# microsoft/NOTSOFAR1-Challenge

Hardware: AMD Instinct MI355X
Metric: CSS real-time-factor (sep. audio sec/wall sec) on 7-ch 16 kHz (higher is better)
Workload: dtype f32 (float32 operands on v_mfma_f32_32x32x2_f32 in every Linear layer, attention product and transform: the reference's own operand precision; MVDR covariance / solve f64)

## Files before the change

### notsofar1-challenge_amd/csrc/api_core.hip

```cpp
#include "api_ctx.hpp"

thread_local std::string g_create_error;

int fail(css_ctx* h, int code, const std::string& msg) {
    if (h) h->err = msg;
    else g_create_error = msg;
    return code;
}

hipError_t dev_alloc(DevBuf& b, size_t bytes) {
    hipError_t e = b.reset();
    if (e == hipSuccess) e = hipMalloc(&b.p, bytes);
    if (e == hipSuccess) b.cap = bytes;
    return e;
}

int ensure(css_ctx* h, DevBuf& b, size_t bytes, bool zero) {
    if (bytes <= b.cap) return CSS_OK;
    if (b.p && h->queued) HIPCHK(h, hipDeviceSynchronize());
    if (const hipError_t e = b.reset()) return fail(h, CSS_ERR_HIP, std::string("hipFree(b.p): ") + hipGetErrorString(e));
    HIPCHK(h, hipMalloc(&b.p, bytes));
    b.cap = bytes;
    if (zero) HIPCHK(h, hipMemsetAsync(b.p, 0, bytes, h->stream));
    return CSS_OK;
// ... 97 lines not shown
    bool ok = true;
    for (int k = 0; k < 20 && ok && !enough(); ++k) {
        hipStream_t st = nullptr;
        if (hipStreamCreateWithFlags(&st, hipStreamNonBlocking) != hipSuccess) { ok = false; break; }
        if (streams_share_a_queue(main, st, e0, e1)) { with_main.push_back(st); continue; }
        bool placed = false;
        for (auto& c : cls)
            if (streams_share_a_queue(c[0], st, e0, e1)) { c.push_back(st); placed = true; break; }
        if (!placed) cls.push_back({st});
    }
    e0.reset();
    e1.reset();
    if (hipGetLastError() != hipSuccess) ok = false;
    std::vector<hipStream_t> take;
    if (ok && !cls.empty()) {
        std::sort(cls.begin(), cls.end(), [](const std::vector<hipStream_t>& x, const std::vector<hipStream_t>& y) { return x.size() > y.size(); });
        auto pop = [&](size_t c) -> hipStream_t {
            for (size_t q = 0; q < cls.size(); ++q) {
                auto& v = cls[(c + q) % cls.size()];
                if (!v.empty()) { hipStream_t s_ = v.back(); v.pop_back(); return s_; }
            }
            if (!with_main.empty()) { hipStream_t s_ = with_main.back(); with_main.pop_back(); return s_; }
            return nullptr;
        };
        const size_t nc = cls.size();
        const size_t cA = 0, cB = nc > 1 ? 1 : 0, cC = nc > 2 ? 2 : cB;
        take.resize(5);
        take[2] = pop(cC);
        take[0] = pop(cA);
        take[1] = pop(cB);
        take[3] = pop(cB);
        take[4] = pop(cA);
        for (hipStream_t s_ : take) ok = ok && s_ != nullptr;
    } else {
        ok = false;
    }
    for (auto& c : cls)
        for (hipStream_t s_ : c) hipStreamDestroy(s_);
    for (hipStream_t s_ : with_main) hipStreamDestroy(s_);
    if (!ok) {
        for (hipStream_t s_ : take)
            if (s_) hipStreamDestroy(s_);
        return false;
    }
    lane[1] = take[0]; lane[2] = take[1]; *copy = take[2]; *tail = take[3]; lane[3] = take[4];
    return true;
}

int plan_impl(const CssModelDesc& d, const CssRunCfg& cfg, int64_t n, CssPlan* p) {
    const int T = cfg.segment_frames, hop = cfg.hop_frames;
    if (T <= 0 || hop <= 0 || hop > T) return CSS_ERR_INVALID_ARG;
    p->n_samples = n;
    p->stft_frames = n < d.frame_len ? 0 : (n - d.frame_len) / d.frame_hop + 1;
    p->mix_frames = std::max<int64_t>(p->stft_frames, T);
    const int64_t ov = T - hop;
    p->num_segments = (p->mix_frames - ov + hop - 1) / hop;
    p->n_out = (p->mix_frames - 1) * d.frame_hop + d.frame_len;
    const int64_t st = (p->num_segments - 1) * hop;
    int64_t en = st + T;
    if (en >= p->mix_frames) en = p->mix_frames;
    p->last_valid = (int32_t)(en - st);
    p->zero_weight = 0;
    if (cfg.w_first && cfg.w_mid && cfg.w_last) {
        for (int64_t t = 0; t < p->mix_frames && !p->zero_weight; ++t) {
            float ws = 0.f;
            for (int64_t seg = std::max<int64_t>(0, (t - T + hop) / hop); seg <= t / hop && seg < p->num_segments; ++seg) {
                const int64_t tl = t - seg * hop;
                if (tl < 0 || tl >= T) continue;
                const float* w = seg == 0 ? cfg.w_first : (seg == p->num_segments - 1 ? cfg.w_last : cfg.w_mid);
                ws += w[tl];
            }
            if (!(ws > 1e-5f)) p->zero_weight = 1;
        }
    }
    return CSS_OK;
}

void gemm(css_ctx* h, const GemmArgs& g, hipStream_t st) {
    CSS_PROF(CSS_PROF_LINEAR, st);
    if (h->profile_gemm) h->gemm_flops += 2.0 * g.M * (double)g.N * g.K * g.batch;
    if (!g.split_in && !g.layout && h->tune[CSS_TUNE_F32_GEMM]) {
        GemmArgs q = g;
        const int t = h->tune[CSS_TUNE_F32_GEMM];
        q.layout = t == 1 ? 2 : (t == 6 ? 1 : 10 + std::min(t - 1, 4));
        launch_gemm(q, st);
        return;
    }
    launch_gemm(g, st);
}

GemmArgs linear(const float* A, int64_t lda, const float* W, int64_t ldw, const float* bias, float* C, int64_t ldc,
                int M, int N, int K, int act) {
    GemmArgs g{};
    g.A = A; g.lda = lda; g.strideA = 0;
    g.B = W; g.ldb = ldw; g.strideB = 0;
    g.C = C; g.ldc = ldc; g.strideC = 0;
    g.M = M; g.N = N; g.K = K; g.batch = 1;
    g.bias = bias; g.bias_along_m = 0; g.act = act;
    g.residual = nullptr; g.ldr = 0; g.alpha = 1.f;
    return g;
}

StitchArgs stitch_args(css_ctx* h) {
    StitchArgs a{};
    const int T = h->cfg.segment_frames;
    a.masks = h->masks_v;
    a.mask_ld = h->mask_ld_v;
    a.sep = (const float*)h->sep.p;
    a.S = h->d.num_spks; a.F = h->d.num_bins; a.T = T; a.hop = h->cfg.hop_frames;
    a.num_segments = h->plan.num_segments; a.T_long = h->plan.mix_frames;
    a.w_first = (const float*)h->segw.p; a.w_mid = a.w_first + T; a.w_last = a.w_mid + T;
    a.perms = (const int32_t*)h->perms.p;
    a.mask_st = (float*)h->mask_st.p; a.activity = (float*)h->activity.p;
    a.act_b = (uint8_t*)h->act_b.p; a.act_tmp = (uint8_t*)h->act_tmp.p; a.act_final = (uint8_t*)h->act_final.p;
    a.activity_th = h->cfg.activity_th; a.dilation = h->cfg.dilation_frames; a.erosion = h->cfg.erosion_frames;
    a.Y = (float*)h->Y.p; a.KIp = h->KIp;
    a.y_split = h->split ? 1 : 0;
    a.level = h->split ? h->peak_dev : nullptr;
    return a;
}

MvdrArgs mvdr_args(css_ctx* h, int64_t lo, int nseg) {
    MvdrArgs a{};
    const int T = h->cfg.segment_frames;
    a.X = (const float*)h->X.p; a.T_ld = h->T_ld; a.stft_frames = h->plan.stft_frames;
    a.C = h->n_ch; a.F = h->d.num_bins;
    a.masks = h->masks_v; a.mask_ld = h->mask_ld_v;
    a.S = h->d.num_spks; a.T = T; a.hop = h->cfg.hop_frames;
    a.seg_lo = lo; a.nseg = nseg;
    a.wta_override = h->have_override ? (const uint8_t*)h->wta.p : nullptr;
    a.scm = (double*)h->scm.p; a.bfw = (double*)h->bfw.p; a.sep = (float*)h->sep.p;
    a.mask_floor = h->cfg.mask_floor;
    a.use_mvdr = (h->n_ch > 1 && h->cfg.mc_mvdr) ? 1 : 0;
    return a;
}

int64_t batch_cap(const css_ctx* h, int T) {
    int64_t cap = h->max_batch;
    const int rows = h->tune[CSS_TUNE_SPLIT_BATCH_ROWS];
    if (h->split && rows > 0 && T > 0) cap = std::min<int64_t>(cap, std::max<int64_t>(1, rows / T));
    return cap;
}

int ensure_activations(css_ctx* h, int64_t nb, int T) {
    const int64_t Mb = nb * T;
    const int D = h->d.attention_dim, FF = h->d.linear_units;
    int rc;
    if ((rc = ensure(h, h->feat, (size_t)Mb * h->Kp * sizeof(float), true)) != CSS_OK) return rc;
    if ((rc = ensure(h, h->hx, (size_t)Mb * D * sizeof(float))) != CSS_OK) return rc;
    if ((rc = ensure(h, h->hu, (size_t)Mb * D * sizeof(float))) != CSS_OK) return rc;
    if ((rc = ensure(h, h->ht, (size_t)Mb * FF * sizeof(float))) != CSS_OK) return rc;
    if ((rc = ensure(h, h->qkv, (size_t)Mb * 3 * D * sizeof(float))) != CSS_OK) return rc;
    if ((rc = ensure(h, h->qkf, (size_t)qk_fragment_floats(nb, T, h->d.attention_heads) * sizeof(float), true)) != CSS_OK) return rc;
    if ((rc = ensure(h, h->ctxb, (size_t)Mb * D * sizeof(float))) != CSS_OK) return rc;
    for (int l = 1; l < h->lanes; ++l) {
        const int64_t M2 = ((nb + 1) / 2) * T;
        if ((rc = ensure(h, h->lfeat[l], (size_t)M2 * h->Kp * sizeof(float), true)) != CSS_OK) return rc;
        if ((rc = ensure(h, h->lhx[l], (size_t)M2 * D * sizeof(float))) != CSS_OK) return rc;
        if ((rc = ensure(h, h->lhu[l], (size_t)M2 * D * sizeof(float))) != CSS_OK) return rc;
        if ((rc = ensure(h, h->lht[l], (size_t)M2 * FF * sizeof(float))) != CSS_OK) return rc;
        if ((rc = ensure(h, h->lqkv[l], (size_t)M2 * 3 * D * sizeof(float))) != CSS_OK) return rc;
        if ((rc = ensure(h, h->lqkf[l], (size_t)qk_fragment_floats(M2 / T, T, h->d.attention_heads) * sizeof(float), true)) != CSS_OK) return rc;
        if ((rc = ensure(h, h->lctx[l], (size_t)M2 * D * sizeof(float))) != CSS_OK) return rc;
    }
    return CSS_OK;
}

// ... 288 lines not shown
    if (!h || lanes < 1 || lanes > css_ctx::MAX_LANES) return fail(h, CSS_ERR_INVALID_ARG, "lanes must be in [1, 4]");
    h->lanes = lanes;
    return CSS_OK;
}

int css_get_lanes(css_handle_t h) { return h ? h->lanes : (int)CSS_ERR_INVALID_ARG; }

int css_set_tuning(css_handle_t h, int which, int value) {
    if (!h || which < 0 || which >= CSS_TUNE_COUNT || value < 0 || (value > 16 && which != CSS_TUNE_SPLIT_BATCH_ROWS && which != CSS_TUNE_F32_LANE_ROWS))
        return fail(h, CSS_ERR_INVALID_ARG, "unknown tuning option / value");
    h->tune[which] = value;
    return CSS_OK;
}

int css_set_range_fallback(css_handle_t h, int enable) {
    if (!h) return CSS_ERR_INVALID_ARG;
    h->range_fallback = enable != 0;
    return CSS_OK;
}

int css_range_status(css_handle_t h, int64_t* fallbacks, int32_t* last_hit) {
    if (!h) return CSS_ERR_INVALID_ARG;
    if (fallbacks) *fallbacks = h->range_fallbacks;
    if (last_hit) *last_hit = h->range_last;
    return CSS_OK;
}

int css_check_range(css_handle_t h) {
    int rc = check_session(h);
    if (rc) return rc;
    HIPCHK(h, hipSetDevice(h->device));
    HIPCHK(h, hipMemcpyAsync(h->range_flag_host.p, h->range_flag_dev.p, sizeof(unsigned int), hipMemcpyDeviceToHost, h->stream));
    HIPCHK(h, hipStreamSynchronize(h->stream));
    if (*h->range_flag_host.as<unsigned int>() && h->split)
        return fail(h, CSS_ERR_RANGE, "an operand of a Linear layer left the split-f16 range (|x| > 65504): use CSS_LINEAR_EXACT_F32");
    return CSS_OK;
}

int css_linear_host(css_handle_t h, const float* x, const float* w, const float* bias, int32_t M, int32_t N, int32_t K,
                    int32_t kernel, int32_t layout, float* y) {
    CSS_DRAIN(h);
    if (!h || !x || !w || !y || M < 1 || N < 1 || K < 32 || K % 32) return fail(h, CSS_ERR_INVALID_ARG, "bad argument (K must be a multiple of 32)");
    if (kernel < 0 || kernel > 2) return fail(h, CSS_ERR_INVALID_ARG, "kernel must be 0 (split, weights direct), 1 (split, LDS staged) or 2 (exact float32)");
    HIPCHK(h, hipSetDevice(h->device));
    const int Np = (N + 31) / 32 * 32;
    const size_t xf = (size_t)M * K, wf = (size_t)Np * K, yf = (size_t)M * N;
    int rc;
    if ((rc = ensure(h, h->stage, (2 * xf + 2 * wf + yf + (size_t)N + 256) * sizeof(float))) != CSS_OK) return rc;
    float* xd = (float*)h->stage.p;
    float* xs = xd + (xf + 15) / 16 * 16;
    float* wd = xs + (xf + 15) / 16 * 16;
    float* ws = wd + (wf + 15) / 16 * 16;
    float* yd = ws + (wf + 15) / 16 * 16;
    float* bd = yd + (yf + 15) / 16 * 16;
    HIPCHK(h, hipMemcpyAsync(xd, x, xf * sizeof(float), hipMemcpyHostToDevice, h->stream));
    HIPCHK(h, hipMemcpyAsync(wd, w, (size_t)N * K * sizeof(float), hipMemcpyHostToDevice, h->stream));
    if (bias) HIPCHK(h, hipMemcpyAsync(bd, bias, (size_t)N * sizeof(float), hipMemcpyHostToDevice, h->stream));
    GemmArgs g = linear(xd, K, wd, K, bias ? bd : nullptr, yd, N, M, N, K, ACT_NONE);
    if (kernel != 2) {
        launch_split_convert(xd, K, xs, M, K, K, h->stream);
        if (kernel == 0) launch_split_convert_tiled(wd, K, ws, N, K, h->stream);
        else launch_split_convert(wd, K, ws, N, K, K, h->stream);
        g.A = xs; g.B = ws; g.split_in = 1; g.b_tiled = kernel == 0;
        if (kernel == 0) g.tile_rows = layout; else g.layout = layout;
    } else {
        g.layout = layout;
    }
    launch_gemm(g, h->stream);
    HIPCHK(h, hipMemcpyAsync(y, yd, yf * sizeof(float), hipMemcpyDeviceToHost, h->stream));
    HIPCHK(h, hipStreamSynchronize(h->stream));
    HIPCHK(h, hipGetLastError());
    return CSS_OK;
}

int css_gemm_host(css_handle_t h, const CssGemmDesc* d, const float* a, const float* b, const float* bias, const float* residual,
                  float* c) {
    CSS_DRAIN(h);
    if (!h) return CSS_ERR_INVALID_ARG;
    auto bad = [&](const char* what) { return fail(h, CSS_ERR_INVALID_ARG, std::string("css_gemm_host: ") + what); };
    if (!d || !a || !b || !c) return bad("null argument");
    const int64_t cap = (int64_t)1 << 28;
    const int M = d->M, N = d->N, K = d->K, batch = d->batch, kernel = d->kernel;
    if (kernel < 0 || kernel > 2) return bad("kernel must be 0 (split, weights direct), 1 (split, LDS staged) or 2 (exact float32)");
    if (M < 1 || N < 1 || batch < 1 || K < 32 || K % 32 || M > (1 << 22) || N > (1 << 22) || K > (1 << 16) || batch > 1024)
        return bad("M, N, batch >= 1 and K a multiple of 32");
    if (d->lda < K || d->ldb < K || d->lda % 4 || d->ldb % 4 || d->lda > cap || d->ldb > cap) return bad("lda, ldb: multiples of 4, at least K");
    if (d->act < ACT_NONE || d->act > ACT_SIGMOID) return bad("act must be 0, 1 or 2");
    if (d->bias < 0 || d->bias > 2 || (d->bias != 0) != (bias != nullptr)) return bad("bias: 0 with NULL, 1 or 2 with an array");
    if (d->residual < 0 || d->residual > 2 || (d->residual == 1) != (residual != nullptr)) return bad("residual: 1 with an array, 0 or 2 with NULL");
    if (!(std::fabs(d->alpha) <= 3.0e38f)) return bad("alpha must be finite");
    if (d->a_off < 0 || d->c_off < 0 || d->r_off < 0 || d->a_off > 1024 || d->c_off > (1 << 20) || d->r_off > 1024) return bad("offsets");
    const bool tr = d->c_transposed != 0, has_res = d->residual != 0;
    const int rows_c = tr ? N : M, cols_c = tr ? M : N;
    if (d->ldc < cols_c || d->ldc > cap) return bad("ldc is shorter than a row of C");
    const int64_t ldr = d->residual == 2 ? d->ldc : d->ldr;
    if (d->residual == 1 && (ldr < N || ldr > cap)) return bad("ldr is shorter than a row of the residual");
    if (d->residual == 2 && batch != 1) return bad("the in-place residual takes batch 1");
    const int64_t extA = (int64_t)(M - 1) * d->lda + K, extB = (int64_t)(N - 1) * d->ldb + K;
    const int64_t extC = (int64_t)(rows_c - 1) * d->ldc + cols_c, extR = (int64_t)(M - 1) * ldr + N;
    const int64_t sA = batch > 1 ? d->strideA : 0, sB = batch > 1 ? d->strideB : 0, sC = batch > 1 ? d->strideC : 0;
    if (sA < 0 || sB < 0 || sA > cap || sB > cap || sC > cap || (sA && sA < extA) || (sB && sB < extB)) return bad("strideA, strideB: 0 or at least one matrix");
    if (batch > 1 && sC < extC) return bad("batch entries of C overlap");
    if (d->a_floats > cap || d->b_floats > cap || d->c_floats > cap || d->r_floats > cap) return bad("an array of more than 2^28 floats");
    if (d->a_floats < d->a_off + (batch - 1) * sA + extA) return bad("a is shorter than its description");
    if (d->b_floats < (batch - 1) * sB + extB) return bad("b is shorter than its description");
    if (d->c_floats < d->c_off + (batch - 1) * sC + extC) return bad("c is shorter than its description");
    if (d->residual == 1 && d->r_floats < d->r_off + extR) return bad("residual is shorter than its description");
    if (d->split_out < 0 || d->split_out % 32 || d->split_out > N || (d->split_out && kernel == 2)) return bad("split_out: a multiple of 32 up to N, kernels 0 and 1");
    if (tr && (kernel != 0 || has_res || d->split_out || d->bias == 2)) return bad("c_transposed: kernel 0, column bias and activation only");
    if (kernel == 0 && (batch != 1 || N % 32)) return bad("kernel 0 takes batch 1 and whole 32-column weight tiles");
    if (kernel == 0 && !tr && (d->c_off % 4 || d->ldc % 4)) return bad("kernel 0 writes 16-byte pieces: c_off and ldc must be multiples of 4");
    if (d->b_frag32 && (kernel != 2 || batch != 1 || N % 32)) return bad("b_frag32: kernel 2, batch 1, N a multiple of 32");
    const int lay = d->layout, tile = d->tile_rows;
    const bool lay_ok = kernel == 0 ? lay == 0
                                    : (lay == 0 || lay == 8 || lay == 4 || lay == 64 || (kernel == 2 && (lay == 1 || lay == 2 || (lay >= 11 && lay <= 14))));
    const bool tile_ok = kernel == 0 ? (tile == 0 || tile == 32 || tile == 64 || tile == 96 || tile == 128 || tile == 4 || tile == 65) : tile == 0;
    if (!lay_ok || !tile_ok) return bad("layout / tile_rows: not a tile layout of this kernel");

    HIPCHK(h, hipSetDevice(h->device));
    auto pad = [](int64_t n) { return (size_t)((n + 63) / 64 * 64); };
    const int nA = sA ? batch : 1, nB = sB ? batch : 1;
    const int Np = (N + 31) / 32 * 32;
    const size_t f_a = pad(d->a_floats), f_b = pad(d->b_floats), f_c = pad(d->c_floats), f_r = pad(d->residual == 1 ? d->r_floats : 0);
    const size_t f_as = kernel != 2 ? pad((int64_t)nA * M * K) : 0, f_bs = kernel == 0 ? pad((int64_t)Np * K) : kernel == 1 ? pad((int64_t)nB * N * K) : 0;
    const size_t f_bf = d->b_frag32 ? pad((int64_t)N * K) : 0, f_bias = pad(d->bias == 2 ? M : N);
    int rc;
    if ((rc = ensure(h, h->stage, (f_a + f_b + f_c + f_r + f_as + f_bs + f_bf + f_bias) * sizeof(float))) != CSS_OK) return rc;
    float* ad = (float*)h->stage.p;
    float* bd = ad + f_a;
    float* cd = bd + f_b;
    float* rd = cd + f_c;
    float* as = rd + f_r;
    float* bs = as + f_as;
    float* bf = bs + f_bs;
    float* biasd = bf + f_bf;
    HIPCHK(h, hipMemcpyAsync(ad, a, (size_t)d->a_floats * sizeof(float), hipMemcpyHostToDevice, h->stream));
    HIPCHK(h, hipMemcpyAsync(bd, b, (size_t)d->b_floats * sizeof(float), hipMemcpyHostToDevice, h->stream));
    HIPCHK(h, hipMemcpyAsync(cd, c, (size_t)d->c_floats * sizeof(float), hipMemcpyHostToDevice, h->stream));
    if (d->residual == 1) HIPCHK(h, hipMemcpyAsync(rd, residual, (size_t)d->r_floats * sizeof(float), hipMemcpyHostToDevice, h->stream));
    if (bias) HIPCHK(h, hipMemcpyAsync(biasd, bias, (size_t)(d->bias == 2 ? M : N) * sizeof(float), hipMemcpyHostToDevice, h->stream));

    GemmArgs g{};
    g.A = ad + d->a_off; g.lda = d->lda; g.strideA = sA;
    g.B = bd; g.ldb = d->ldb; g.strideB = sB;
    g.C = cd + d->c_off; g.ldc = d->ldc; g.strideC = sC;
    g.M = M; g.N = N; g.K = K; g.batch = batch;
    g.bias = bias ? biasd : nullptr; g.bias_along_m = d->bias == 2; g.act = d->act;
    g.residual = d->residual == 1 ? rd + d->r_off : d->residual == 2 ? g.C : nullptr;
    g.ldr = has_res ? ldr : 0; g.alpha = has_res ? d->alpha : 1.f;
    g.split_out = d->split_out; g.c_transposed = tr; g.m_fastest = d->m_fastest != 0; g.nt_store = d->nt_store != 0;
    g.concurrent = d->concurrent != 0;
    if (kernel != 2) {
        for (int z = 0; z < nA; ++z) launch_split_convert(g.A + z * sA, d->lda, as + (int64_t)z * M * K, M, K, K, h->stream);
        if (kernel == 0) launch_split_convert_tiled(bd, d->ldb, bs, N, K, h->stream);
        else for (int z = 0; z < nB; ++z) launch_split_convert(bd + z * sB, d->ldb, bs + (int64_t)z * N * K, N, K, K, h->stream);
        g.A = as; g.lda = K; g.strideA = sA ? (int64_t)M * K : 0;
        g.B = bs; g.ldb = K; g.strideB = sB ? (int64_t)N * K : 0;
        g.split_in = 1; g.b_tiled = kernel == 0;
        g.tile_rows = tile; g.layout = lay;
    } else {
        g.layout = lay;
        if (d->b_frag32) {
            launch_f32_fragments(bd, d->ldb, bf, N, K, h->stream);
            g.B = bf; g.b_frag32 = 1; g.B_rows = bd;
        }
    }
    launch_gemm(g, h->stream);
    HIPCHK(h, hipMemcpyAsync(c, cd, (size_t)d->c_floats * sizeof(float), hipMemcpyDeviceToHost, h->stream));
    HIPCHK(h, hipStreamSynchronize(h->stream));
    HIPCHK(h, hipGetLastError());
    return CSS_OK;
}

int css_host_alloc(size_t bytes, void** out) {
    if (!out) return CSS_ERR_INVALID_ARG;
    *out = nullptr;
    return hipHostMalloc(out, bytes ? bytes : 1, hipHostMallocDefault) == hipSuccess ? CSS_OK : CSS_ERR_HIP;
}

int css_host_free(void* p) { return (!p || hipHostFree(p) == hipSuccess) ? CSS_OK : CSS_ERR_HIP; }

int css_set_linear_mode(css_handle_t h, int mode) {
    CSS_DRAIN(h);
    if (!h || (mode != CSS_LINEAR_SPLIT_F16 && mode != CSS_LINEAR_EXACT_F32)) return fail(h, CSS_ERR_INVALID_ARG, "unknown linear mode");
    const bool split = mode == CSS_LINEAR_SPLIT_F16;
    if (split == h->split) return CSS_OK;
    if (split && stream_open_count(h)) return fail(h, CSS_ERR_STATE, "a stream is open: streams run in CSS_LINEAR_EXACT_F32 only");
    if (split && !h->split_ok) return fail(h, CSS_ERR_RANGE, "a weight of this model lies outside the split-f16 operand range (|w| > 65504)");
    HIPCHK(h, hipSetDevice(h->device));
    if (split) {
        int rc = make_split_weights(h);
        if (rc) return rc;
    } else if (make_frag_weights(h) != CSS_OK) {
        (void)hipGetLastError();
        h->wfrag.reset();
    }
    if (h->feat.p) HIPCHK(h, hipMemsetAsync(h->feat.p, 0, h->feat.cap, h->stream));
    for (int l = 1; l < css_ctx::MAX_LANES; ++l)
// ... 342 lines not shown
```

### notsofar1-challenge_amd/csrc/gemm.hip

```cpp
#include <cstdlib>

#include <cstdio>

#include "gemm_common.hpp"

namespace css {

template <int BM, int WM>
__global__ __launch_bounds__(WM * 128, 2) void gemm_kernel(GemmArgs g, int tiles_m, int tiles_n) {
    constexpr int THREADS = WM * 128;
    constexpr int TM = (BM / WM) / 32;
    constexpr int LROWS = THREADS / 8;
    constexpr int NLA = BM / LROWS;
    constexpr int NLB = BN / LROWS;
    static_assert((NLA == 2 || NLA == 4) && (NLB == 2 || NLB == 4) && (TM == 1 || TM == 2), "unsupported tile layout");
    __shared__ __attribute__((aligned(16))) float lds[2 * (BM + BN) * LDS_LD];
    const int n_tiles = tiles_m * tiles_n * g.batch;
    const int L = blockIdx.x;
    const int tile = xcd_tile(L, n_tiles);
    const int per_batch = tiles_m * tiles_n;
    const int bz = tile / per_batch;
    const int t2 = tile - bz * per_batch;
    const int tn = g.m_fastest ? t2 / tiles_m : t2 % tiles_n, tm = g.m_fastest ? t2 % tiles_m : t2 / tiles_n;
    const int m0 = tm * BM, n0 = tn * BN;
// ... 37 lines not shown
#define CSS_LSTORE(buf)                                                         \
    {                                                                           \
        float* as_ = lds + (buf) * (BM + BN) * LDS_LD + lr * LDS_LD + lc;       \
        float* bs_ = as_ + BM * LDS_LD;                                         \
        *reinterpret_cast<float4*>(as_) = ra0;                                  \
        *reinterpret_cast<float4*>(as_ + LROWS * LDS_LD) = ra1;                 \
        *reinterpret_cast<float4*>(bs_) = rb0;                                  \
        *reinterpret_cast<float4*>(bs_ + LROWS * LDS_LD) = rb1;                 \
        if constexpr (NLA == 4) {                                               \
            *reinterpret_cast<float4*>(as_ + 2 * LROWS * LDS_LD) = ra2;         \
            *reinterpret_cast<float4*>(as_ + 3 * LROWS * LDS_LD) = ra3;         \
        }                                                                       \
        if constexpr (NLB == 4) {                                               \
            *reinterpret_cast<float4*>(bs_ + 2 * LROWS * LDS_LD) = rb2;         \
            *reinterpret_cast<float4*>(bs_ + 3 * LROWS * LDS_LD) = rb3;         \
        }                                                                       \
    }

    f32x16 acc00 = {0}, acc01 = {0}, acc10 = {0}, acc11 = {0};
    const int nk = g.K / BK;
    CSS_GLOAD(0)
    CSS_LSTORE(0)
    __syncthreads();
    for (int kt = 0; kt < nk; ++kt) {
        const int buf = kt & 1;
        if (kt + 1 < nk) { CSS_GLOAD((kt + 1) * BK) }
        const float* as = lds + buf * (BM + BN) * LDS_LD + (wm * (BM / WM) + c) * LDS_LD + 4 * h;
        const float* bs = lds + buf * (BM + BN) * LDS_LD + BM * LDS_LD + (wn * 64 + c) * LDS_LD + 4 * h;
#pragma unroll
        for (int ch = 0; ch < 4; ++ch) {
            const float4 a0 = *reinterpret_cast<const float4*>(as + ch * 8);
            const float4 b0 = *reinterpret_cast<const float4*>(bs + ch * 8);
            const float4 b1 = *reinterpret_cast<const float4*>(bs + 32 * LDS_LD + ch * 8);
            float4 a1 = a0;
            if constexpr (TM == 2) a1 = *reinterpret_cast<const float4*>(as + 32 * LDS_LD + ch * 8);
#define CSS_MFMA_STEP(e)                                                                 \
    acc00 = __builtin_amdgcn_mfma_f32_32x32x2f32(a0.e, b0.e, acc00, 0, 0, 0);            \
    acc01 = __builtin_amdgcn_mfma_f32_32x32x2f32(a0.e, b1.e, acc01, 0, 0, 0);            \
    if constexpr (TM == 2) {                                                             \
        acc10 = __builtin_amdgcn_mfma_f32_32x32x2f32(a1.e, b0.e, acc10, 0, 0, 0);        \
        acc11 = __builtin_amdgcn_mfma_f32_32x32x2f32(a1.e, b1.e, acc11, 0, 0, 0);        \
    }
            CSS_MFMA_STEP(x) CSS_MFMA_STEP(y) CSS_MFMA_STEP(z) CSS_MFMA_STEP(w)
#undef CSS_MFMA_STEP
        }
        if (kt + 1 < nk) CSS_LSTORE(buf ^ 1)
        __syncthreads();
    }
#undef CSS_GLOAD
#undef CSS_LSTORE

    const float* bias = g.bias;
    const float* res = g.residual;
    const int act = g.act, bias_m = g.bias_along_m;
    const int64_t ldc = g.ldc, ldr = g.ldr;
    const float alpha = g.alpha;
    const int mrow = m0 + wm * (BM / WM) + 4 * h, ncol = n0 + wn * 64 + c;
    const bool wide = (ldc % 4 == 0) && (N % 4 == 0) && ((reinterpret_cast<uintptr_t>(C) & 15) == 0);
    if (wide) {
        __syncthreads();
        float* patch = lds + wave * (32 * LDS_LD);
        const int mt = m0 + wm * (BM / WM), nt = n0 + wn * 64;
        emit_tile_wide(acc00, mt, h, c, nt, M, N, C, ldc, bias, bias_m, act, res, ldr, alpha, 0, patch);
        emit_tile_wide(acc01, mt, h, c, nt + 32, M, N, C, ldc, bias, bias_m, act, res, ldr, alpha, 0, patch);
        if constexpr (TM == 2) {
            emit_tile_wide(acc10, mt + 32, h, c, nt, M, N, C, ldc, bias, bias_m, act, res, ldr, alpha, 0, patch);
            emit_tile_wide(acc11, mt + 32, h, c, nt + 32, M, N, C, ldc, bias, bias_m, act, res, ldr, alpha, 0, patch);
        }
        return;
    }
    emit_tile(acc00, mrow, ncol, M, N, C, ldc, bias, bias_m, act, res, ldr, alpha, 0);
    emit_tile(acc01, mrow, ncol + 32, M, N, C, ldc, bias, bias_m, act, res, ldr, alpha, 0);
    if constexpr (TM == 2) {
        emit_tile(acc10, mrow + 32, ncol, M, N, C, ldc, bias, bias_m, act, res, ldr, alpha, 0);
        emit_tile(acc11, mrow + 32, ncol + 32, M, N, C, ldc, bias, bias_m, act, res, ldr, alpha, 0);
    }
}

void launch_gemm(const GemmArgs& g_in, hipStream_t s) {
    if (g_in.M <= 0 || g_in.N <= 0 || g_in.batch <= 0 || g_in.K <= 0) return;
    if (g_in.split_in) return g_in.b_tiled ? launch_gemm_split_wd(g_in, s) : launch_gemm_split(g_in, s);
    GemmArgs g = g_in;
    int forced = g.layout;
    if (forced == 0 || forced == 1 || (forced >= 11 && forced <= 14)) {
        if (launch_gemm_f32(g, s, forced >= 11 ? forced - 10 : 0)) return;
        forced = 0;
    }
    if (g.b_frag32) {
        if (!g.B_rows) {
            fprintf(stderr, "css_mi355: launch_gemm: a fragment-ordered weight (b_frag32) reached the row-major kernel without B_rows "
                            "(M %d N %d K %d layout %d): launch dropped\n", g.M, g.N, g.K, g.layout);
            return;
        }
        g.B = g.B_rows;
        g.b_frag32 = 0;
    }
    if (forced == 2) forced = 0;
    const int tiles_n = (g.N + BN - 1) / BN;
    const int blocks128 = ((g.M + 127) / 128) * tiles_n * g.batch;
    int layout = forced ? forced : (blocks128 < 1000 ? 8 : 4);
    if (!forced) {
        const double waste128 = (double)(((g.M + 127) / 128) * 128 - g.M) / g.M;
        const double waste64 = (double)(((g.M + 63) / 64) * 64 - g.M) / g.M;
        if (waste128 - waste64 > 0.03) layout = 64;
    }
    if (layout == 64) {
        const int tiles_m = (g.M + 63) / 64;
        hipLaunchKernelGGL((gemm_kernel<64, 2>), dim3(tiles_m * tiles_n * g.batch), dim3(256), 0, s, g, tiles_m, tiles_n);
    } else if (layout == 8) {
        const int tiles_m = (g.M + 127) / 128;
        hipLaunchKernelGGL((gemm_kernel<128, 4>), dim3(blocks128), dim3(512), 0, s, g, tiles_m, tiles_n);
    } else {
        const int tiles_m = (g.M + 127) / 128;
        hipLaunchKernelGGL((gemm_kernel<128, 2>), dim3(blocks128), dim3(256), 0, s, g, tiles_m, tiles_n);
    }
}

}
```

### notsofar1-challenge_amd/csrc/gemm_f32.hip

```cpp
#include <algorithm>
#include <type_traits>

#include "gemm_common.hpp"

namespace css {

namespace {

constexpr int F_BK = 16;
constexpr int F_LD = 20;
constexpr int F_BUF = (128 + BN) * F_LD;
constexpr int F_PATCH_LD = 36;

typedef float f32x4 __attribute__((ext_vector_type(4)));

__device__ __forceinline__ float epi_value(float acc, float bn, float bm, int act, bool has_res, float rv, float alpha) {
    float v = acc + bn + bm;
    if (act == ACT_RELU) v = fmaxf(v, 0.f);
    else if (act == ACT_SIGMOID) v = sigmoidf_(v);
    if (has_res) v = rv + alpha * v;
    return v;
}

template <int TM, bool BD, bool FAST>
// ... 285 lines not shown
                F32_AFTER_STORE(o)
#if F32_TRANSPOSED >= 2
                __builtin_amdgcn_sched_barrier(0);
                asm volatile("s_nop 7");
#if F32_TRANSPOSED >= 3
                asm volatile("s_nop 7");
#endif
                __builtin_amdgcn_sched_barrier(0);
#endif
            }
        }
        F32_EPILOGUE_PROBE
        return;
    }
#else
    if constexpr (FAST) {
        const int voC = (int)(((unsigned)(m0 + erow) * (unsigned)ldc + n) * 4u);
        auto epilogue = [&](auto relu_c, auto res_c) {
            const bool relu = relu_c;
            constexpr bool res = decltype(res_c)::value;
#pragma unroll
            for (int i = 0; i < TM; ++i) {
#pragma unroll
                for (int r = 0; r < 16; ++r) patch[((r & 3) + 8 * (r >> 2) + 4 * h) * F_PATCH_LD + c] = acc[i][r];
                if (i + 1 < TM && res) prefetch_fast(i + 1, (i + 1) & 1, lane_e);
#pragma unroll
                for (int j = 0; j < 4; ++j) {
                    const f32x4 v = *reinterpret_cast<const f32x4*>(patch + (erow + 8 * j) * F_PATCH_LD + col4);
                    f32x4 o;
#pragma unroll
                    for (int e = 0; e < 4; ++e) {
                        float t = v[e] + bn[e];
                        if (relu) t = fmaxf(t, 0.f);
                        if (res) t = rv[i & 1][j][e] + alpha * t;
                        o[e] = t;
                    }
                    typedef unsigned int u32x4 __attribute__((ext_vector_type(4)));
                    __builtin_amdgcn_raw_buffer_store_b128(__builtin_bit_cast(u32x4, o), rsC, voC, (int)((unsigned)(32 * i + 8 * j) * (unsigned)ldc * 4u), 0);
                    F32_AFTER_STORE(o)
                }
            }
        };
        if (has_res) epilogue(act == ACT_RELU, std::true_type{});
        else if (act == ACT_RELU) epilogue(std::true_type{}, std::false_type{});
        else epilogue(std::false_type{}, std::false_type{});
        F32_EPILOGUE_PROBE
        return;
    }
#endif
#pragma unroll
    for (int i = 0; i < TM; ++i) {
#if F32_TRANSPOSED
#pragma unroll
        for (int q = 0; q < 4; ++q)
            *reinterpret_cast<f32x4*>(patch + c * F_PATCH_LD + 8 * q + 4 * h) = f32x4{acc[i][4 * q], acc[i][4 * q + 1], acc[i][4 * q + 2], acc[i][4 * q + 3]};
#else
#pragma unroll
        for (int r = 0; r < 16; ++r) patch[((r & 3) + 8 * (r >> 2) + 4 * h) * F_PATCH_LD + c] = acc[i][r];
#endif
        if (i + 1 < TM) prefetch(i + 1, (i + 1) & 1, lane_e);
#pragma unroll
        for (int j = 0; j < 4; ++j) {
            const int row = erow + 8 * j, m = m0 + 32 * i + row;
            const f32x4 v = *reinterpret_cast<const f32x4*>(patch + row * F_PATCH_LD + col4);
            if (m >= M || !col_ok) continue;
            float* dst = C + (int64_t)m * ldc + n;
            const float bm = bias_m ? bias[m] : 0.f;
            f32x4 o;
#pragma unroll
            for (int e = 0; e < 4; ++e) o[e] = epi_value(v[e], bn[e], bm, act, has_res, rv[i & 1][j][e], alpha);
            if (wide) {
                *reinterpret_cast<f32x4*>(dst) = o;
            } else {
#pragma unroll
                for (int e = 0; e < 4; ++e)
                    if (n + e < N) dst[e] = o[e];
            }
        }
    }
    F32_EPILOGUE_PROBE
#undef F32_EPILOGUE_PROBE
}

}

struct F32Plan {
    int u, tiles_n, ncu, max_tm; int64_t U;
#if F32_TOOLS
    unsigned long long* dbg;
#endif
};

template <bool BD, bool FAST>
__global__ __launch_bounds__(256, 4) void gemm_f32_kernel(GemmArgs g, F32Plan p) {
    __shared__ __attribute__((aligned(16))) float lds[2 * F_BUF];
    const int b = blockIdx.x, v = b % p.ncu, j = b / p.ncu;
    const int64_t lo = p.U * v / p.ncu, hi = p.U * (v + 1) / p.ncu;
    int64_t pos = lo + (hi - lo) * j / 4;
    const int64_t end = lo + (hi - lo) * (j + 1) / 4;
    int want = std::min(1 + (b + j) % 4, p.max_tm);
    bool first = true;
#if F32_TOOLS
    if (p.dbg && threadIdx.x == 0) {
        p.dbg[4 * b + 0] = wall_clock64();
        p.dbg[4 * b + 2] = ((unsigned long long)__builtin_amdgcn_s_getreg(63508) << 32) | (unsigned)__builtin_amdgcn_s_getreg(63492);
        p.dbg[4 * b + 3] = __builtin_readcyclecounter();
    }
#endif
    const int64_t panel0 = pos / p.u;
    int r = (int)(pos - panel0 * p.u);
    int bz = (int)(panel0 / p.tiles_n), tn = (int)(panel0 - (int64_t)bz * p.tiles_n);
    while (pos < end) {
        const int tm = (int)std::min<int64_t>(std::min<int64_t>(want, end - pos), p.u - r);
        const float* A = g.A + (int64_t)bz * g.strideA;
        const float* B = g.B + (int64_t)bz * g.strideB;
        float* C = g.C + (int64_t)bz * g.strideC;
        if (!first) __syncthreads();
        first = false;
        switch (tm) {
            case 1: f32_tile<1, BD, FAST>(g, A, B, C, 32 * r, tn * BN, lds); break;
            case 2: f32_tile<2, BD, FAST>(g, A, B, C, 32 * r, tn * BN, lds); break;
            case 3: f32_tile<3, BD, FAST>(g, A, B, C, 32 * r, tn * BN, lds); break;
            default: f32_tile<4, BD, FAST>(g, A, B, C, 32 * r, tn * BN, lds); break;
        }
        pos += tm;
        want = p.max_tm;
        r += tm;
        if (r == p.u) {
            r = 0;
            if (++tn == p.tiles_n) { tn = 0; ++bz; }
        }
    }
#if F32_TOOLS
    if (p.dbg && threadIdx.x == 0) { p.dbg[4 * b + 1] = wall_clock64(); p.dbg[4 * b + 3] = __builtin_readcyclecounter() - p.dbg[4 * b + 3]; }
#endif
}

static bool f32_fast_epilogue(const GemmArgs& g) {
    const int64_t lim = (int64_t)1 << 31;
    const bool has_res = g.residual != nullptr;
    const bool wide = (g.ldc % 4 == 0) && (g.N % 4 == 0) && ((reinterpret_cast<uintptr_t>(g.C) & 15) == 0) &&
                      (g.batch == 1 || g.strideC % 4 == 0) &&
                      (!has_res || ((g.ldr % 4 == 0) && ((reinterpret_cast<uintptr_t>(g.residual) & 15) == 0)));
    return F32_FAST_EPILOGUE && wide && !(g.bias && g.bias_along_m) && (g.N % BN == 0) && g.act != ACT_SIGMOID &&
           (int64_t)g.M * g.ldc * 4 < lim && (!has_res || (int64_t)g.M * g.ldr * 4 < lim);
}

bool launch_gemm_f32(const GemmArgs& g, hipStream_t s, int forced_tm) {
    if (g.M <= 0 || g.N <= 0 || g.batch <= 0) return true;
    if (g.K <= 0 || g.K % F_BK) return false;
    const int64_t lim = (int64_t)1 << 31;
    if ((((int64_t)g.M + 128) * g.lda + g.K) * 4 >= lim || (((int64_t)g.N + 128) * g.ldb + g.K) * 4 >= lim) return false;
    if (g.b_frag32 && (g.N % 32 || g.K % 16 || g.batch != 1 || ((int64_t)g.N * g.K * 4 >= lim))) return false;
    if ((g.lda % 4) || (!g.b_frag32 && (g.ldb % 4)) || (reinterpret_cast<uintptr_t>(g.A) & 15) || (reinterpret_cast<uintptr_t>(g.B) & 15)) return false;
    constexpr int NCU = 256;
    F32Plan p;
    p.u = (g.M + 31) / 32;
    p.tiles_n = (g.N + BN - 1) / BN;
    p.ncu = NCU;
    p.max_tm = (forced_tm >= 1 && forced_tm <= 4) ? forced_tm : 4;
    p.U = (int64_t)p.u * p.tiles_n * g.batch;
#if F32_TOOLS
    p.dbg = g.narrow_epilogue == 77 ? reinterpret_cast<unsigned long long*>(g.range_flag) : nullptr;
#endif
    const bool fast = f32_fast_epilogue(g);
    void (*kern)(GemmArgs, F32Plan) = g.b_frag32 ? (fast ? gemm_f32_kernel<true, true> : gemm_f32_kernel<true, false>)
                                                 : (fast ? gemm_f32_kernel<false, true> : gemm_f32_kernel<false, false>);
    hipLaunchKernelGGL(kern, dim3(4 * NCU), dim3(256), 0, s, g, p);
    return true;
}


__global__ void f32_fragments_kernel(const float* __restrict__ src, int64_t ld_src, float* __restrict__ dst, int N, int K) {
    const int64_t idx = (int64_t)blockIdx.x * blockDim.x + threadIdx.x;
    const int64_t total = (int64_t)(N / 32) * (K / 8) * 64;
    if (idx >= total) return;
    const int lane = (int)(idx & 63);
    const int64_t t = idx >> 6;
    const int kc = (int)(t % (K / 8)), j = (int)(t / (K / 8));
    const float* p = src + (int64_t)(32 * j + (lane & 31)) * ld_src + 8 * kc + 4 * (lane >> 5);
    reinterpret_cast<float4*>(dst)[idx] = make_float4(p[0], p[1], p[2], p[3]);
}
void launch_f32_fragments(const float* src, int64_t ld_src, float* dst, int N, int K, hipStream_t s) {
    const int64_t total = (int64_t)(N / 32) * (K / 8) * 64;
    if (total <= 0) return;
    hipLaunchKernelGGL(f32_fragments_kernel, dim3((unsigned)((total + 255) / 256)), dim3(256), 0, s, src, ld_src, dst, N, K);
}

}
```

Measured before the change: 7364.

## Add wide 256-column f32 MFMA GEMM tile kernel with A-ahead double buffering

Adds a new f32 GEMM kernel that computes 256-column output tiles per block, with four waves each owning 64 columns. It reads pre-fragmented weights straight from global memory into registers and double-buffers A in LDS, prefetching the next-next A chunk. The kernel is picked automatically for b_frag32 GEMMs with a fast epilogue when M is below a threshold and the wide grid needs at most half as many block rounds as the narrow one. Wider tiles reuse each A load across more columns, at the cost of more accumulator registers (2 blocks per CU) and coarser load balance. New tune layouts 17/18/21-24 and relaxed K checks are exposed in the host API.

```diff
diff --git a/notsofar1-challenge_amd/csrc/api_core.hip b/notsofar1-challenge_amd/csrc/api_core.hip
--- a/notsofar1-challenge_amd/csrc/api_core.hip
+++ b/notsofar1-challenge_amd/csrc/api_core.hip
@@ -203,7 +203,7 @@
     if (!g.split_in && !g.layout && h->tune[CSS_TUNE_F32_GEMM]) {
         GemmArgs q = g;
         const int t = h->tune[CSS_TUNE_F32_GEMM];
-        q.layout = t == 1 ? 2 : (t == 6 ? 1 : 10 + std::min(t - 1, 4));
+        q.layout = t == 1 ? 2 : (t == 6 ? 1 : (t == 7 ? 17 : (t == 8 ? 18 : 10 + std::min(t - 1, 4))));
         launch_gemm(q, st);
         return;
     }
@@ -658,7 +658,12 @@
     const int64_t cap = (int64_t)1 << 28;
     const int M = d->M, N = d->N, K = d->K, batch = d->batch, kernel = d->kernel;
     if (kernel < 0 || kernel > 2) return bad("kernel must be 0 (split, weights direct), 1 (split, LDS staged) or 2 (exact float32)");
-    if (M < 1 || N < 1 || batch < 1 || K < 32 || K % 32 || M > (1 << 22) || N > (1 << 22) || K > (1 << 16) || batch > 1024)
+    const bool f32_only = kernel == 2 && (d->layout == 17 || d->layout == 18 || (d->layout >= 21 && d->layout <= 24));
+    const int64_t f32_lim = (int64_t)1 << 29;
+    const bool f32_takes = d->a_off % 4 == 0 && d->lda > 0 && d->ldb > 0 && d->lda < f32_lim && d->ldb < f32_lim && M > 0 && N > 0 && K > 0 &&
+                           ((int64_t)M + 128) * d->lda + K < f32_lim && ((int64_t)N + 128) * d->ldb + K < f32_lim;
+    const int kstep = f32_only && f32_takes ? 16 : 32;
+    if (M < 1 || N < 1 || batch < 1 || K < kstep || K % kstep || M > (1 << 22) || N > (1 << 22) || K > (1 << 16) || batch > 1024)
         return bad("M, N, batch >= 1 and K a multiple of 32");
     if (d->lda < K || d->ldb < K || d->lda % 4 || d->ldb % 4 || d->lda > cap || d->ldb > cap) return bad("lda, ldb: multiples of 4, at least K");
     if (d->act < ACT_NONE || d->act > ACT_SIGMOID) return bad("act must be 0, 1 or 2");
@@ -689,7 +694,7 @@
     if (d->b_frag32 && (kernel != 2 || batch != 1 || N % 32)) return bad("b_frag32: kernel 2, batch 1, N a multiple of 32");
     const int lay = d->layout, tile = d->tile_rows;
     const bool lay_ok = kernel == 0 ? lay == 0
-                                    : (lay == 0 || lay == 8 || lay == 4 || lay == 64 || (kernel == 2 && (lay == 1 || lay == 2 || (lay >= 11 && lay <= 14))));
+                                    : (lay == 0 || lay == 8 || lay == 4 || lay == 64 || (kernel == 2 && (lay == 1 || lay == 2 || (lay >= 11 && lay <= 14) || lay == 17 || lay == 18 || (lay >= 21 && lay <= 24))));
     const bool tile_ok = kernel == 0 ? (tile == 0 || tile == 32 || tile == 64 || tile == 96 || tile == 128 || tile == 4 || tile == 65) : tile == 0;
     if (!lay_ok || !tile_ok) return bad("layout / tile_rows: not a tile layout of this kernel");
 
diff --git a/notsofar1-challenge_amd/csrc/gemm.hip b/notsofar1-challenge_amd/csrc/gemm.hip
--- a/notsofar1-challenge_amd/csrc/gemm.hip
+++ b/notsofar1-challenge_amd/csrc/gemm.hip
@@ -143,8 +143,8 @@
     if (g_in.split_in) return g_in.b_tiled ? launch_gemm_split_wd(g_in, s) : launch_gemm_split(g_in, s);
     GemmArgs g = g_in;
     int forced = g.layout;
-    if (forced == 0 || forced == 1 || (forced >= 11 && forced <= 14)) {
-        if (launch_gemm_f32(g, s, forced >= 11 ? forced - 10 : 0)) return;
+    if (forced == 0 || forced == 1 || (forced >= 11 && forced <= 14) || forced == 17 || forced == 18 || (forced >= 21 && forced <= 24)) {
+        if (launch_gemm_f32(g, s, forced >= 21 ? forced - 20 : (forced >= 11 && forced <= 14) ? forced - 10 : 0)) return;
         forced = 0;
     }
     if (g.b_frag32) {
diff --git a/notsofar1-challenge_amd/csrc/gemm_f32.hip b/notsofar1-challenge_amd/csrc/gemm_f32.hip
--- a/notsofar1-challenge_amd/csrc/gemm_f32.hip
+++ b/notsofar1-challenge_amd/csrc/gemm_f32.hip
@@ -391,6 +391,225 @@
 #undef F32_EPILOGUE_PROBE
 }
 
+constexpr int W_BN = 256;
+constexpr int W_BUF = 128 * F_LD;
+#ifndef F32W_AHEAD
+#define F32W_AHEAD 1
+#endif
+
+template <int TM>
+__device__ __forceinline__ void f32w_tile(const GemmArgs& g, const float* __restrict__ A, const float* __restrict__ B,
+                                          float* __restrict__ C, const int m0, const int n0, float* __restrict__ lds) {
+    const int tid = threadIdx.x, lane = tid & 63, w = tid >> 6, c = lane & 31, h = lane >> 5;
+    const int M = g.M, N = g.N;
+    constexpr int BM = 32 * TM;
+    constexpr int NPA = (BM + 63) / 64;
+    constexpr int NLD = NPA + 4;
+    const int srow = tid >> 2, sk = (tid & 3) * 4;
+    const int64_t extA = (int64_t)(M - 1) * g.lda + (g.lda > g.K ? g.lda : g.K);
+    const __amdgpu_buffer_rsrc_t rsA = __builtin_amdgcn_make_buffer_rsrc(const_cast<float*>(A), 0, (int)(extA * 4), 0x00020000);
+    const __amdgpu_buffer_rsrc_t rsB = __builtin_amdgcn_make_buffer_rsrc(const_cast<float*>(B), 0, (int)((int64_t)N * g.K * 4), 0x00020000);
+    const int voA = (int)(((int64_t)(m0 + srow) * g.lda + sk) * 4);
+    const int passA = (int)(64 * g.lda * 4);
+    const bool a1_on = (BM % 64 == 0) || srow < BM % 64;
+    const int vw = (int)((((int64_t)(n0 / 32 + 2 * w) * (g.K / 8)) * 64 + lane) * 16);
+    const int tstep = (g.K / 8) * 1024;
+    f32x4 ra[NPA], wc[2][2], wn[2][2];
+#if F32W_AHEAD
+    f32x4 ra2[NPA];
+#endif
+    const int nk = g.K / F_BK;
+    auto load_a = [&](f32x4 (&r)[NPA], int k0, int i) {
+        if (i + 1 < NPA || a1_on) r[i] = __builtin_bit_cast(f32x4, __builtin_amdgcn_raw_buffer_load_b128(rsA, voA, k0 * 4 + i * passA, 0));
+    };
+    auto load_w = [&](int k0, int q) {
+        wn[q >> 1][q & 1] = __builtin_bit_cast(f32x4, __builtin_amdgcn_raw_buffer_load_b128(rsB, vw, (k0 / 8 + (q & 1)) * 1024 + (q >> 1) * tstep, 0));
+    };
+    auto store_a = [&](const f32x4 (&r)[NPA], int buf) {
+        float* as_ = lds + buf * W_BUF + srow * F_LD + sk;
+#pragma unroll
+        for (int i = 0; i < NPA; ++i) {
+            if (i + 1 < NPA || a1_on) *reinterpret_cast<f32x4*>(as_ + i * 64 * F_LD) = r[i];
+        }
+    };
+    f32x16 acc[TM][2];
+#pragma unroll
+    for (int i = 0; i < TM; ++i) { acc[i][0] = f32x16{0}; acc[i][1] = f32x16{0}; }
+#if F32_PROBE
+    const unsigned long long t_in_ = (w == 0) ? __builtin_readcyclecounter() : 0;
+#endif
+#pragma unroll
+    for (int i = 0; i < NPA; ++i) load_a(ra, 0, i);
+#pragma unroll
+    for (int q = 0; q < 4; ++q) load_w(0, q);
+#if F32W_AHEAD
+    if (nk > 1) {
+#pragma unroll
+        for (int i = 0; i < NPA; ++i) load_a(ra2, F_BK, i);
+    }
+#endif
+    store_a(ra, 0);
+#pragma unroll
+    for (int q = 0; q < 4; ++q) wc[q >> 1][q & 1] = wn[q >> 1][q & 1];
+    __syncthreads();
+    const int aoff = c * F_LD + 4 * h;
+
+    const float* __restrict__ bias = g.bias;
+    const float* __restrict__ res = g.residual;
+    const int act = g.act;
+    const bool has_res = res != nullptr;
+    const unsigned ldc = (unsigned)g.ldc, ldr = (unsigned)g.ldr;
+    const float alpha = g.alpha;
+    const __amdgpu_buffer_rsrc_t rsR = __builtin_amdgcn_make_buffer_rsrc(const_cast<float*>(res), 0, has_res ? (int)((unsigned)M * ldr * 4u) : 0, 0x00020000);
+    f32x4 rv[2][4];
+    auto prefetch_fast = [&](int s, int slot, int lane_) {
+        const int vo_ = (int)(((unsigned)(m0 + (lane_ >> 3)) * ldr + n0 + 64 * w + 32 * (s & 1) + (lane_ & 7) * 4) * 4u);
+#pragma unroll
+        for (int j = 0; j < 4; ++j)
+            rv[slot][j] = __builtin_bit_cast(f32x4, __builtin_amdgcn_raw_buffer_load_b128(rsR, vo_, (int)((unsigned)(32 * (s >> 1) + 8 * j) * ldr * 4u), 0));
+    };
+
+    auto compute = [&](int buf, int k0n, auto ahead_c) {
+        constexpr bool a_ahead = decltype(ahead_c)::value;
+        const float* as = lds + buf * W_BUF + aoff;
+#pragma unroll
+        for (int ch = 0; ch < 2; ++ch) {
+            f32x4 a[TM];
+#pragma unroll
+            for (int i = 0; i < TM; ++i) a[i] = *reinterpret_cast<const f32x4*>(as + i * 32 * F_LD + 8 * ch);
+            __builtin_amdgcn_sched_barrier(0);
+#pragma unroll
+            for (int e = 0; e < 4; ++e) {
+                const int q = ch * 4 + e;
+                if (k0n >= 0 && q < NLD) {
+                    if constexpr (a_ahead) {
+#if F32W_AHEAD
+                        if (q < 4) load_w(k0n, q);
+                        else load_a(ra2, k0n + F_BK, q - 4);
+#endif
+                    } else {
+                        if (q < NPA) load_a(ra, k0n, q);
+                        else load_w(k0n, q - NPA);
+                    }
+                    __builtin_amdgcn_sched_barrier(0);
+                }
+#pragma unroll
+                for (int i = 0; i < TM; ++i) {
+#pragma unroll
+                    for (int t = 0; t < 2; ++t) acc[i][t] = __builtin_amdgcn_mfma_f32_32x32x2f32(a[i][e], wc[t][ch][e], acc[i][t], 0, 0, 0);
+                }
+                if (k0n >= 0) __builtin_amdgcn_sched_barrier(0);
+            }
+            __builtin_amdgcn_sched_barrier(0);
+        }
+    };
+#if F32_PROBE
+    const bool probe = w == 0 && g.narrow_epilogue == 77 && g.range_flag;
+    unsigned long long pc_ = 0, pl_ = 0, pb_ = 0, pt_ = 0;
+    const unsigned long long t_loop_ = probe ? __builtin_readcyclecounter() : 0;
+#define F32_CLK(var) if (probe) var = __builtin_readcyclecounter();
+#else
+#define F32_CLK(var)
+#endif
+    for (int kt = 0; kt + 1 < nk; ++kt) {
+#if F32_PROBE
+        unsigned long long t0_ = 0, t1_ = 0, t2_ = 0, t3_ = 0;
+#endif
+        F32_CLK(t0_)
+#if F32W_AHEAD
+        store_a(ra2, (kt + 1) & 1);
+        __builtin_amdgcn_sched_barrier(0);
+        F32_CLK(t1_)
+        compute(kt & 1, (kt + 1) * F_BK, std::true_type{});
+        F32_CLK(t2_)
+#else
+        __builtin_amdgcn_sched_barrier(0);
+        compute(kt & 1, (kt + 1) * F_BK, std::false_type{});
+        F32_CLK(t1_)
+        store_a(ra, (kt + 1) & 1);
+        F32_CLK(t2_)
+#endif
+#pragma unroll
+        for (int q = 0; q < 4; ++q) wc[q >> 1][q & 1] = wn[q >> 1][q & 1];
+        __syncthreads();
+        F32_CLK(t3_)
+#if F32_PROBE
+#if F32W_AHEAD
+        pl_ += t1_ - t0_; pc_ += t2_ - t1_; pb_ += t3_ - t2_; pt_ += 1;
+#else
+        pc_ += t1_ - t0_; pl_ += t2_ - t1_; pb_ += t3_ - t2_; pt_ += 1;
+#endif
+#endif
+    }
+#if F32_PROBE
+    if (probe && lane == 0) {
+        unsigned long long* pr = reinterpret_cast<unsigned long long*>(g.range_flag) + 4096 + 4 * blockIdx.x;
+        atomicAdd(pr + 0, pc_); atomicAdd(pr + 1, pl_); atomicAdd(pr + 2, pb_); atomicAdd(pr + 3, pt_);
+        atomicAdd(pr + 4096 + 0, t_loop_ - t_in_);
+        atomicAdd(pr + 4096 + 1, 1ull);
+    }
+    const unsigned long long t_out_ = probe ? __builtin_readcyclecounter() : 0;
+#endif
+#undef F32_CLK
+    {
+        int lane_ = lane;
+        asm volatile("" : "+v"(lane_));
+        if (has_res) prefetch_fast(0, 0, lane_);
+    }
+    compute((nk - 1) & 1, -1, std::false_type{});
+    __syncthreads();
+
+    int lane_e = lane;
+    asm volatile("" : "+v"(lane_e));
+    float* patch = lds + w * (32 * F_PATCH_LD);
+    const int col4 = (lane_e & 7) * 4, n = n0 + 64 * w + col4, erow = lane_e >> 3;
+    float bn[2][4] = {{0.f, 0.f, 0.f, 0.f}, {0.f, 0.f, 0.f, 0.f}};
+    if (bias) {
+#pragma unroll
+        for (int t = 0; t < 2; ++t) {
+#pragma unroll
+            for (int e = 0; e < 4; ++e) bn[t][e] = bias[n + 32 * t + e];
+        }
+    }
+    const int voC = (int)(((unsigned)(m0 + erow) * ldc + n) * 4u);
+    const __amdgpu_buffer_rsrc_t rsC = __builtin_amdgcn_make_buffer_rsrc(C, 0, (int)((unsigned)M * ldc * 4u), 0x00020000);
+    auto epilogue = [&](auto relu_c, auto res_c) {
+        const bool relu = relu_c;
+        constexpr bool with_res = decltype(res_c)::value;
+#pragma unroll
+        for (int s = 0; s < 2 * TM; ++s) {
+            const int i = s >> 1, t = s & 1;
+#pragma unroll
+            for (int r = 0; r < 16; ++r) patch[((r & 3) + 8 * (r >> 2) + 4 * h) * F_PATCH_LD + c] = acc[i][t][r];
+            if (s + 1 < 2 * TM && with_res) prefetch_fast(s + 1, (s + 1) & 1, lane_e);
+#pragma unroll
+            for (int j = 0; j < 4; ++j) {
+                const f32x4 v = *reinterpret_cast<const f32x4*>(patch + (erow + 8 * j) * F_PATCH_LD + col4);
+                f32x4 o;
+#pragma unroll
+                for (int e = 0; e < 4; ++e) {
+                    float x = v[e] + bn[t][e];
+                    if (relu) x = fmaxf(x, 0.f);
+                    if (with_res) x = rv[s & 1][j][e] + alpha * x;
+                    o[e] = x;
+                }
+                typedef unsigned int u32x4 __attribute__((ext_vector_type(4)));
+                __builtin_amdgcn_raw_buffer_store_b128(__builtin_bit_cast(u32x4, o), rsC, voC, (int)(((unsigned)(32 * i + 8 * j) * ldc + 32 * t) * 4u), 0);
+                F32_AFTER_STORE(o)
+            }
+        }
+    };
+    if (has_res) epilogue(act == ACT_RELU, std::true_type{});
+    else if (act == ACT_RELU) epilogue(std::true_type{}, std::false_type{});
+    else epilogue(std::false_type{}, std::false_type{});
+#if F32_PROBE
+    if (probe && lane == 0) {
+        unsigned long long* pr = reinterpret_cast<unsigned long long*>(g.range_flag) + 4096 + 4 * blockIdx.x;
+        atomicAdd(pr + 4096 + 2, __builtin_readcyclecounter() - t_out_);
+    }
+#endif
+}
+
 }
 
 struct F32Plan {
@@ -445,6 +664,42 @@
 #endif
 }
 
+__global__ __launch_bounds__(256, 2) void gemm_f32_wide_kernel(GemmArgs g, F32Plan p) {
+    __shared__ __attribute__((aligned(16))) float lds[2 * W_BUF];
+    const int b = blockIdx.x, v = b % p.ncu, j = b / p.ncu;
+    const int lo = (int)(p.U * v / p.ncu), hi = (int)(p.U * (v + 1) / p.ncu);
+    int pos = lo + (hi - lo) * j / 2;
+    const int end = lo + (hi - lo) * (j + 1) / 2;
+    int want = std::min(1 + (b + j) % 4, p.max_tm);
+    bool first = true;
+#if F32_TOOLS
+    if (p.dbg && threadIdx.x == 0) {
+        p.dbg[4 * b + 0] = wall_clock64();
+        p.dbg[4 * b + 2] = ((unsigned long long)__builtin_amdgcn_s_getreg(63508) << 32) | (unsigned)__builtin_amdgcn_s_getreg(63492);
+        p.dbg[4 * b + 3] = __builtin_readcyclecounter();
+    }
+#endif
+    int tn = pos / p.u, r = pos - tn * p.u;
+    while (pos < end) {
+        const int tm = std::min(std::min(want, end - pos), p.u - r);
+        if (!first) __syncthreads();
+        first = false;
+        switch (tm) {
+            case 1: f32w_tile<1>(g, g.A, g.B, g.C, 32 * r, tn * W_BN, lds); break;
+            case 2: f32w_tile<2>(g, g.A, g.B, g.C, 32 * r, tn * W_BN, lds); break;
+            case 3: f32w_tile<3>(g, g.A, g.B, g.C, 32 * r, tn * W_BN, lds); break;
+            default: f32w_tile<4>(g, g.A, g.B, g.C, 32 * r, tn * W_BN, lds); break;
+        }
+        pos += tm;
+        want = p.max_tm;
+        r += tm;
+        if (r == p.u) { r = 0; ++tn; }
+    }
+#if F32_TOOLS
+    if (p.dbg && threadIdx.x == 0) { p.dbg[4 * b + 1] = wall_clock64(); p.dbg[4 * b + 3] = __builtin_readcyclecounter() - p.dbg[4 * b + 3]; }
+#endif
+}
+
 static bool f32_fast_epilogue(const GemmArgs& g) {
     const int64_t lim = (int64_t)1 << 31;
     const bool has_res = g.residual != nullptr;
@@ -455,6 +710,18 @@
            (int64_t)g.M * g.ldc * 4 < lim && (!has_res || (int64_t)g.M * g.ldr * 4 < lim);
 }
 
+#ifndef F32_WIDE_MAX_M
+#define F32_WIDE_MAX_M 24576
+#endif
+static bool f32_wide_choice(const GemmArgs& g, bool fast) {
+    if (!g.b_frag32 || !fast || g.N % W_BN) return false;
+    if (g.layout == 17 || (g.layout >= 21 && g.layout <= 24)) return true;
+    if (g.layout != 0 && g.layout != 1) return false;
+    if (g.M >= F32_WIDE_MAX_M) return false;
+    const int64_t u = (g.M + 31) / 32, wide_units = u * (g.N / W_BN), narrow_units = u * (g.N / BN);
+    return 2 * ((wide_units + 255) / 256) <= (narrow_units + 255) / 256;
+}
+
 bool launch_gemm_f32(const GemmArgs& g, hipStream_t s, int forced_tm) {
     if (g.M <= 0 || g.N <= 0 || g.batch <= 0) return true;
     if (g.K <= 0 || g.K % F_BK) return false;
@@ -463,6 +730,20 @@
     if (g.b_frag32 && (g.N % 32 || g.K % 16 || g.batch != 1 || ((int64_t)g.N * g.K * 4 >= lim))) return false;
     if ((g.lda % 4) || (!g.b_frag32 && (g.ldb % 4)) || (reinterpret_cast<uintptr_t>(g.A) & 15) || (reinterpret_cast<uintptr_t>(g.B) & 15)) return false;
     constexpr int NCU = 256;
+    const bool fast = f32_fast_epilogue(g);
+    if (f32_wide_choice(g, fast)) {
+        F32Plan p;
+        p.u = (g.M + 31) / 32;
+        p.tiles_n = g.N / W_BN;
+        p.ncu = NCU;
+        p.max_tm = (forced_tm >= 1 && forced_tm <= 4) ? forced_tm : 4;
+        p.U = (int64_t)p.u * p.tiles_n;
+#if F32_TOOLS
+        p.dbg = g.narrow_epilogue == 77 ? reinterpret_cast<unsigned long long*>(g.range_flag) : nullptr;
+#endif
+        hipLaunchKernelGGL(gemm_f32_wide_kernel, dim3(2 * NCU), dim3(256), 0, s, g, p);
+        return true;
+    }
     F32Plan p;
     p.u = (g.M + 31) / 32;
     p.tiles_n = (g.N + BN - 1) / BN;
@@ -472,7 +753,6 @@
 #if F32_TOOLS
     p.dbg = g.narrow_epilogue == 77 ? reinterpret_cast<unsigned long long*>(g.range_flag) : nullptr;
 #endif
-    const bool fast = f32_fast_epilogue(g);
     void (*kern)(GemmArgs, F32Plan) = g.b_frag32 ? (fast ? gemm_f32_kernel<true, true> : gemm_f32_kernel<true, false>)
                                                  : (fast ? gemm_f32_kernel<false, true> : gemm_f32_kernel<false, false>);
     hipLaunchKernelGGL(kern, dim3(4 * NCU), dim3(256), 0, s, g, p);
```

Result: no change. 7308 (-0.8%).
